# Ruyi-Zha/r2_gaussian

Hardware: NVIDIA H100
Metric: projections_per_sec (higher is better)
Workload: dtype f32

## Files before the change

### r2_gaussian_b200/csrc/r2x_api.cu

```cuda
#include <atomic>
#include <cstdio>
#include <cstring>
#include <string>
#include "../../include/r2x.h"
#include "r2x_binning.cuh"
#include "r2x_raster.cuh"
#include "r2x_voxel.cuh"

namespace r2x {
int launch_adam(cudaStream_t st, int ngroups, const r2x_adam_group* groups, double beta1, double beta2, double eps,
                long long step, const float* const* grads2, const uint32_t* guard0, const uint32_t* guard1);
int launch_densify_stats(cudaStream_t st, int P, const int* radii, const float* grad2d, float* max_radii, float* accum,
                         float* denom, const uint32_t* guard0, const uint32_t* guard1);

static thread_local std::string g_err;
static thread_local Activation g_act = {0, 0, 0.f, 0.f};
Activation current_activation() { return g_act; }
void set_activation(const Activation* a) { g_act = a ? *a : Activation{0, 0, 0.f, 0.f}; }

int fail(cudaError_t e, const char* what, const char* file, int line) {
    char buf[512];
    snprintf(buf, sizeof(buf), "CUDA error %d (%s) at %s:%d: %s", (int)e, cudaGetErrorString(e), file, line, what);
    g_err = buf;
    return R2X_ERR_CUDA;
// ... 227 lines not shown
    uint2* ranges = (uint2*)al((size_t)image_buf);
    if (P == 0) {
        R2X_CUDA_OK(cudaMemsetAsync(out_color, 0, sizeof(float) * (size_t)W * H, st));
        R2X_CUDA_OK(cudaMemsetAsync(ranges, 0, sizeof(uint2) * tiles, st));
        R2X_CUDA_OK(cudaMemsetAsync(s.status, 0, 16, st));
        if (status_dev) R2X_CUDA_OK(cudaMemsetAsync(status_dev, 0, 8, st));
        return 0;
    }
    if (!means3D || !opacities || !radii || !viewmatrix || !projmatrix)
        return fail_msg(R2X_ERR_INVALID, "r2x_raster_forward: null input");
    if (!cov3D_precomp && (!scales || !rotations))
        return fail_msg(R2X_ERR_INVALID, "r2x_raster_forward: need scales+rotations or cov3D_precomp");
    const bool direct = direct_ok(tiles);
    DirectBin db{};
    if (direct) {
        db = carve_directbin(image_buf, P, tiles);
    }
    R2X_TRY(launch_raster_preprocess(st, P, means3D, scales, scale_modifier, rotations, opacities, cov3D_precomp,
                                     viewmatrix, projmatrix, W, H, tan_fovx, tan_fovy, mode, prefiltered, radii,
                                     s.geom, direct ? &db : nullptr));
    R2X_TRY(debug_sync(st, debug, "raster preprocess"));
    if (direct) {
        const long long cap0 = binning_alloc ? (1ll << 62) : capacity;
        R2X_TRY(launch_direct_scan(st, db, s.status, cap0, binning_alloc ? nullptr : status_dev));
    } else {
        R2X_TRY(launch_scan(st, P, s.geom.tiles_touched, s.geom.offsets, s.scan_state, s.status));
    }
    R2X_TRY(debug_sync(st, debug, "raster scan"));
    long long R_launch;
    if (binning_alloc) {
        uint32_t R = 0;
        R2X_CUDA_OK(cudaMemcpyAsync(&R, s.status, sizeof(uint32_t), cudaMemcpyDeviceToHost, st));
        R2X_CUDA_OK(cudaStreamSynchronize(st));
        if (num_rendered) *num_rendered = (int)R;
        binning_buf = binning_alloc(binning_bytes((long long)R), alloc_user);
        if (!binning_buf) return fail_msg(R2X_ERR_INVALID, "r2x_raster_forward: binning allocator returned NULL");
        capacity = R;
        R_launch = R;
    } else {
        if (!binning_buf || capacity < 0) return fail_msg(R2X_ERR_INVALID, "r2x_raster_forward_async: no binning buffer");
        R_launch = capacity;
    }
    BinningView bv = binning_view(binning_buf, capacity);
    const TilePlan plan = carve_plan(image_buf, tiles, bv);
    if (direct) {
        R2X_TRY(launch_direct_fill(st, P, s.geom.cube, s.geom.tiles_touched, s.geom.offsets, db, ranges, plan, bv,
                                   s.geom.gx, s.geom.gy, s.status));
    } else {
        status_kernel<<<1, 1, 0, st>>>(s.status, capacity, status_dev);
        R2X_TRY(bin_instances(st, P, s.geom.cube, s.geom.tiles_touched, s.geom.offsets, s.geom.gx, s.geom.gy, tiles,
                              s.status, bv, R_launch, ranges));
        R2X_TRY(launch_plan(st, ranges, plan));
    }
    R2X_TRY(debug_sync(st, debug, "raster binning"));
    R2X_TRY(launch_raster_render(st, W, H, s.geom, ranges, bv.point_list, plan, R_launch, out_color));
    R2X_TRY(debug_sync(st, debug, "raster render"));
    return 0;
}

int voxel_forward_impl(cudaStream_t st, int P, int nx, int ny, int nz, float sx, float sy, float sz, float cx,
                       float cy, float cz, const float* means3D, const float* opacities, const float* scales,
                       float scale_modifier, const float* rotations, const float* cov3D_precomp, int prefiltered,
                       float* out_volume, int* radii_x, int* radii_y, int* radii_z, void* geom_buf, void* image_buf,
                       r2x_alloc_fn binning_alloc, void* alloc_user, void* binning_buf, long long capacity,
                       uint32_t* status_dev, int debug, int* num_rendered) {
    (void)prefiltered;
    if (nx <= 0 || ny <= 0 || nz <= 0 || P < 0) return fail_msg(R2X_ERR_INVALID, "r2x_voxel_forward: bad P/grid");
    if (!out_volume || !geom_buf || !image_buf) return fail_msg(R2X_ERR_INVALID, "r2x_voxel_forward: null output/state buffer");
    if (num_rendered) *num_rendered = 0;
    const VoxelGrid vg = make_voxel_grid(nx, ny, nz, sx, sy, sz, cx, cy, cz);
// ... 8 lines not shown
        R2X_CUDA_OK(cudaMemsetAsync(ranges, 0, sizeof(uint2) * (size_t)tiles, st));
        R2X_CUDA_OK(cudaMemsetAsync(s.status, 0, 16, st));
        if (status_dev) R2X_CUDA_OK(cudaMemsetAsync(status_dev, 0, 8, st));
        return 0;
    }
    if (!means3D || !opacities || !radii_x || !radii_y || !radii_z)
        return fail_msg(R2X_ERR_INVALID, "r2x_voxel_forward: null input");
    if (!scales)
        return fail_msg(R2X_ERR_INVALID,
                        "r2x_voxel_forward: scales are required (the bounding radius is 3*max(scale)/dVoxel even "
                        "with cov3D_precomp; the reference dereferences scales unconditionally, VOX/forward.cu:137)");
    if (!cov3D_precomp && !rotations) return fail_msg(R2X_ERR_INVALID, "r2x_voxel_forward: need rotations or cov3D_precomp");
    const bool direct = direct_ok(tiles);
    const bool two_level = two_level_ok(vg.gx, vg.gy, vg.gz);
    DirectBin db{};
    if (direct) {
        db = carve_directbin(image_buf, P, tiles);
    }
    R2X_TRY(launch_voxel_preprocess(st, P, means3D, scales, scale_modifier, rotations, opacities, cov3D_precomp, vg,
                                    radii_x, radii_y, radii_z, s.geom, direct ? &db : nullptr));
    R2X_TRY(debug_sync(st, debug, "voxel preprocess"));
    if (direct) {
        const long long cap0 = binning_alloc ? (1ll << 62) : capacity;
        R2X_TRY(launch_direct_scan(st, db, s.status, cap0, binning_alloc ? nullptr : status_dev));
    } else {
        R2X_TRY(launch_scan(st, P, s.geom.tiles_touched, s.geom.offsets, s.scan_state, s.status));
    }
    long long R_launch;
    if (binning_alloc) {
        uint32_t R = 0;
        R2X_CUDA_OK(cudaMemcpyAsync(&R, s.status, sizeof(uint32_t), cudaMemcpyDeviceToHost, st));
        R2X_CUDA_OK(cudaStreamSynchronize(st));
        if (num_rendered) *num_rendered = (int)R;
        binning_buf = binning_alloc(binning_bytes((long long)R), alloc_user);
        if (!binning_buf) return fail_msg(R2X_ERR_INVALID, "r2x_voxel_forward: binning allocator returned NULL");
        capacity = R;
        R_launch = R;
    } else {
        if (!binning_buf || capacity < 0) return fail_msg(R2X_ERR_INVALID, "r2x_voxel_forward_async: no binning buffer");
        R_launch = capacity;
    }
    BinningView bv = binning_view(binning_buf, capacity);
    const TilePlan plan = carve_voxel_plan(image_buf, tiles, bv);
    if (direct) {
        R2X_TRY(launch_direct_fill(st, P, s.geom.cube, s.geom.tiles_touched, s.geom.offsets, db, ranges, plan, bv, vg.gx,
                                   vg.gy, s.status));
    } else if (two_level) {
        status_kernel<<<1, 1, 0, st>>>(s.status, capacity, status_dev);
        const TwoLevel tl = carve_two_level(image_buf, P, vg.gx, vg.gy, vg.gz, bv);
        R2X_TRY(launch_two_level(st, P, s.geom.cube, s.geom.tiles_touched, vg.gx, vg.gy, vg.gz, s.status, tl, bv, ranges,
                                 plan));
    } else {
        status_kernel<<<1, 1, 0, st>>>(s.status, capacity, status_dev);
        R2X_TRY(bin_instances(st, P, s.geom.cube, s.geom.tiles_touched, s.geom.offsets, vg.gx, vg.gy, tiles, s.status,
                              bv, R_launch, ranges));
        R2X_TRY(launch_plan(st, ranges, plan));
    }
    R2X_TRY(debug_sync(st, debug, "voxel binning"));
    R2X_TRY(launch_voxel_render(st, vg, s.geom, ranges, bv.point_list, plan, R_launch, out_volume));
    R2X_TRY(debug_sync(st, debug, "voxel render"));
    return 0;
}

}
}

using namespace r2x;

extern "C" {
// ... 322 lines not shown
```

### r2_gaussian_b200/csrc/r2x_binning.cu

```cuda
#include <cstdlib>
#include "r2x_binning.cuh"

namespace r2x {

static inline size_t align_up(size_t v, size_t a) { return (v + a - 1) / a * a; }

static size_t plan_items(long long R) { return (size_t)(R > 0 ? R : 1) / PLAN_MIN_CHUNK + 1; }

int plan_chunk_override() {
    static int v = -1;
    if (v < 0) {
        const char* e = getenv("R2X_CHUNK");
        v = e ? atoi(e) : 0;
        if (v < 0) v = 0;
    }
    return v;
}

size_t binning_bytes(long long R) {
    size_t r = (size_t)(R > 0 ? R : 1);
    size_t per = align_up(r * sizeof(uint32_t), 256);
    return 7 * per + align_up(256 * SORT_MAX_BLOCKS * sizeof(uint32_t), 256) +
           align_up(plan_items(R) * sizeof(uint2), 256) + align_up(plan_items(R) * 512 * sizeof(float), 256) + 256;
}
// ... 416 lines not shown
    }
}

__global__ void __launch_bounds__(256) tile_ranges_kernel(const uint32_t* __restrict__ keys,
                                                          const uint32_t* __restrict__ d_total,
                                                          long long capacity, uint2* __restrict__ ranges) {
    long long R = *d_total;
    if (R > capacity) R = capacity;
    const long long stride = (long long)gridDim.x * blockDim.x;
    for (long long i = (long long)blockIdx.x * blockDim.x + threadIdx.x; i < R; i += stride) {
        const uint32_t cur = keys[i];
        if (i == 0) ranges[cur].x = 0;
        else {
            const uint32_t prev = keys[i - 1];
            if (cur != prev) { ranges[prev].y = (uint32_t)i; ranges[cur].x = (uint32_t)i; }
        }
        if (i == R - 1) ranges[cur].y = (uint32_t)R;
    }
}

size_t directbin_bytes(int P, int num_tiles) {
    const size_t nb = (size_t)((P > 0 ? P : 1) + DIRECT_BLOCK - 1) / DIRECT_BLOCK;
    const size_t t = (size_t)num_tiles;
    return align_up(t * nb * sizeof(uint32_t), 256) + align_up(t * sizeof(uint32_t), 256) +
           2 * align_up(nb * sizeof(uint32_t), 256) + 512;
}

DirectBin directbin_view(void* buf, int P, int num_tiles) {
    DirectBin db;
    const size_t nb = (size_t)((P > 0 ? P : 1) + DIRECT_BLOCK - 1) / DIRECT_BLOCK;
    const size_t t = (size_t)num_tiles;
    char* p = (char*)align_up((size_t)buf, 256);
    db.table = (uint32_t*)p; p += align_up(t * nb * sizeof(uint32_t), 256);
    db.tile_count = (uint32_t*)p; p += align_up(t * sizeof(uint32_t), 256);
    db.block_total = (uint32_t*)p; p += align_up(nb * sizeof(uint32_t), 256);
    db.block_base = (uint32_t*)p; p += align_up(nb * sizeof(uint32_t), 256);
    db.num_tiles = num_tiles;
    db.nb = (int)nb;
    return db;
}

template <typename Load, typename Store>
__device__ __forceinline__ uint32_t cta_exclusive_scan(int n, Load load, Store store, uint32_t* s_w, uint32_t* s_carry) {
    const int tid = threadIdx.x, lane = tid & 31, warp = tid >> 5;
    if (tid == 0) *s_carry = 0;
    __syncthreads();
    for (int base = 0; base < n; base += 256) {
        const int i = base + tid;
        const uint32_t a = i < n ? load(i) : 0u;
        uint32_t ia = a;
#pragma unroll
        for (int o = 1; o < 32; o <<= 1) {
            const uint32_t t = __shfl_up_sync(0xffffffffu, ia, o);
            if (lane >= o) ia += t;
        }
        if (lane == 31) s_w[warp] = ia;
        __syncthreads();
        uint32_t wpre = 0;
#pragma unroll
        for (int w = 0; w < 8; ++w)
            if (w < warp) wpre += s_w[w];
        const uint32_t ex = *s_carry + wpre + ia - a;
        if (i < n) store(i, ex, a);
        __syncthreads();
        if (tid == 255) *s_carry = ex + a;
        __syncthreads();
    }
    return *s_carry;
}

template <typename V, typename Load, typename Store>
__device__ __forceinline__ V cta_exclusive_scan_1pass(int n, Load load, Store store, V* s_w) {
    const int tid = threadIdx.x, lane = tid & 31, warp = tid >> 5;
    const int K = (n + 255) >> 8;
    V val[16], sum = 0;
#pragma unroll
    for (int k = 0; k < 16; ++k) {
        const int i = tid * K + k;
        val[k] = (k < K && i < n) ? load(i) : V(0);
        sum += val[k];
    }
    V ia = sum;
#pragma unroll
    for (int o = 1; o < 32; o <<= 1) {
        const V t = __shfl_up_sync(0xffffffffu, ia, o);
        if (lane >= o) ia += t;
    }
    __syncthreads();
    if (lane == 31) s_w[warp] = ia;
    __syncthreads();
    V wpre = 0, total = 0;
#pragma unroll
    for (int w = 0; w < 8; ++w) {
        const V x = s_w[w];
        if (w < warp) wpre += x;
        total += x;
    }
    V ex = wpre + ia - sum;
#pragma unroll
    for (int k = 0; k < 16; ++k) {
        const int i = tid * K + k;
        if (k < K && i < n) store(i, ex, val[k], total);
        ex += val[k];
    }
    return total;
}

constexpr int SCAN_SEGS = 32;
__global__ void __launch_bounds__(1024) direct_scan_kernel(DirectBin db, uint32_t* __restrict__ status,
                                                           long long capacity, uint32_t* __restrict__ status_out) {
    pdl_prologue();
    __shared__ uint32_t s_seg[SCAN_SEGS][33];
    __shared__ uint32_t s_red[32];
    const int lane = threadIdx.x & 31, seg = threadIdx.x >> 5;
    const int T = db.num_tiles, nb = db.nb;
    const int t = blockIdx.x * 32 + lane;
    const int rps = (nb + SCAN_SEGS - 1) / SCAN_SEGS;
    const int r0 = min(seg * rps, nb), r1 = min(r0 + rps, nb);
    uint32_t sum = 0;
    if (t < T) {
        const uint32_t* col = db.table + t;
        int r = r0;
        for (; r + 4 <= r1; r += 4) {
            const uint32_t a0 = col[(size_t)r * T], a1 = col[(size_t)(r + 1) * T], a2 = col[(size_t)(r + 2) * T],
                           a3 = col[(size_t)(r + 3) * T];
            sum += (a0 + a1) + (a2 + a3);
        }
        for (; r < r1; ++r) sum += col[(size_t)r * T];
    }
    s_seg[seg][lane] = sum;
    __syncthreads();
    uint32_t pre = 0;
    for (int k = 0; k < seg; ++k) pre += s_seg[k][lane];
    if (t < T) {
        if (seg == SCAN_SEGS - 1) db.tile_count[t] = pre + sum;
        uint32_t* col = db.table + t;
        int r = r0;
        for (; r + 4 <= r1; r += 4) {
            const uint32_t a0 = col[(size_t)r * T], a1 = col[(size_t)(r + 1) * T], a2 = col[(size_t)(r + 2) * T],
                           a3 = col[(size_t)(r + 3) * T];
            col[(size_t)r * T] = pre;
            col[(size_t)(r + 1) * T] = pre + a0;
            col[(size_t)(r + 2) * T] = pre + a0 + a1;
            col[(size_t)(r + 3) * T] = pre + a0 + a1 + a2;
            pre += (a0 + a1) + (a2 + a3);
        }
        for (; r < r1; ++r) {
            const uint32_t a = col[(size_t)r * T];
            col[(size_t)r * T] = pre;
            pre += a;
        }
    }
    if (blockIdx.x == 0) {
        __shared__ uint32_t s_carry;
        if (threadIdx.x == 0) s_carry = 0;
        __syncthreads();
        for (int base = 0; base < nb; base += 1024) {
            const int i = base + threadIdx.x;
            const uint32_t a = i < nb ? db.block_total[i] : 0u;
            uint32_t ia = a;
#pragma unroll
            for (int o = 1; o < 32; o <<= 1) {
                const uint32_t x = __shfl_up_sync(0xffffffffu, ia, o);
                if (lane >= o) ia += x;
            }
            if (lane == 31) s_red[seg] = ia;
            __syncthreads();
            uint32_t wpre = 0;
            for (int w = 0; w < seg; ++w) wpre += s_red[w];
            const uint32_t ex = s_carry + wpre + ia - a;
            if (i < nb) db.block_base[i] = ex;
            __syncthreads();
            if (threadIdx.x == 1023) s_carry = ex + a;
            __syncthreads();
        }
        if (threadIdx.x == 0) {
            const uint32_t R = s_carry;
            const uint32_t ov = ((long long)R > capacity) ? 1u : 0u;
            status[0] = R;
            status[1] = ov;
            if (status_out) { status_out[0] = R; status_out[1] = ov; }
        }
    }
}

int launch_direct_scan(cudaStream_t st, const DirectBin& db, uint32_t* status, long long capacity,
                       uint32_t* status_out) {
    R2X_CUDA_OK(pdl_launch(direct_scan_kernel, dim3((db.num_tiles + 31) / 32), dim3(1024), 0, st, db, status, capacity,
                           status_out));
    R2X_CUDA_OK(cudaGetLastError());
    return 0;
}

__global__ void __launch_bounds__(DIRECT_BLOCK) direct_fill_kernel(int P, const uint16_t* __restrict__ cube,
                                                                   const uint32_t* __restrict__ tiles_touched,
                                                                   uint32_t* __restrict__ offsets, DirectBin db,
                                                                   uint2* __restrict__ ranges, TilePlan pl,
                                                                   uint32_t* __restrict__ point_list,
                                                                   uint32_t* __restrict__ inst_pos, long long capacity,
                                                                   int gx, int gy, const uint32_t* __restrict__ status) {
    pdl_prologue();
    extern __shared__ __align__(16) unsigned char smem_raw[];
    __shared__ unsigned long long s_w[8];
    const int T = db.num_tiles;
    const int tid = threadIdx.x, lane = tid & 31, warp = tid >> 5;
    const uint32_t* tc = db.tile_count;
    uint32_t* s_mask = reinterpret_cast<uint32_t*>(smem_raw);
    uint32_t* s_base = s_mask + 8 * (size_t)T;
    unsigned char* s_wrank = reinterpret_cast<unsigned char*>(s_base + T);
    __shared__ uint32_t s_w8[8];

    const int b = blockIdx.x;
    const int g = b * DIRECT_BLOCK + tid;
    for (int i = tid; i < 2 * T; i += DIRECT_BLOCK) reinterpret_cast<uint4*>(s_mask)[i] = make_uint4(0u, 0u, 0u, 0u);
    uint32_t n = 0, c01 = 0, c23 = 0, c45 = 0;
    if (g < P) {
        n = tiles_touched[g];
        const uint32_t* c = reinterpret_cast<const uint32_t*>(cube + 6 * (size_t)g);
        c01 = c[0]; c23 = c[1]; c45 = c[2];
    }
    const uint32_t bbase = db.block_base[b];
    uint32_t ia = n;
#pragma unroll
    for (int o = 1; o < 32; o <<= 1) {
        const uint32_t x = __shfl_up_sync(0xffffffffu, ia, o);
        if (lane >= o) ia += x;
    }
    if (lane == 31) s_w8[warp] = ia;
    const uint32_t* row = db.table + (size_t)b * T;
    const uint32_t C = plan_chunk_for(status[0], pl.chunk_override, pl.chunk_cap);
    const int npub = db.nb < DIRECT_BLOCK ? db.nb : DIRECT_BLOCK;
    const bool pub = (b < npub) && (tid % npub == b);
    const unsigned long long tot = cta_exclusive_scan_1pass<unsigned long long>(
        T,
        [&](int i) {
            const uint32_t c = tc[i];
            return ((unsigned long long)(c ? (c - 1) / C : 0u) << 32) | c;
        },
        [&](int i, unsigned long long ex64, unsigned long long v64, unsigned long long total) {
            const uint32_t ex = (uint32_t)ex64, cnt = (uint32_t)v64;
            s_base[i] = ex + row[i];
            if (pub) {
                const bool ov = (long long)(uint32_t)total > capacity;
                const uint32_t eo = ov ? 0u : (uint32_t)(ex64 >> 32), ne = ov ? 0u : (uint32_t)(v64 >> 32);
                ranges[i] = ov ? make_uint2(0u, 0u) : make_uint2(ex, ex + cnt);
                pl.extra_off[i] = eo;
#pragma unroll
                for (int k = 0; k < PLAN_DONE_SLOTS; ++k) pl.tile_done[(size_t)i * PLAN_DONE_SLOTS + k] = 0;
                for (uint32_t c = 0; c < ne; ++c)
                    if ((long long)(eo + c) < pl.max_extra) pl.extra_item[eo + c] = make_uint2((uint32_t)i, c + 1);
            }
        },
        s_w);
    const uint32_t R = (uint32_t)tot;
    if (b == 0 && tid == 0) {
        pl.extra_off[T] = ((long long)R > capacity) ? 0u : (uint32_t)(tot >> 32);
        pl.counter[0] = pl.counter[1] = pl.counter[3] = 0;
        pl.counter[2] = C;
    }
    uint32_t wpre = 0;
#pragma unroll
    for (int w = 0; w < 8; ++w)
        if (w < warp) wpre += s_w8[w];
    const uint32_t lex = wpre + ia - n;
    if (g < P) offsets[g] = bbase + lex + n;
    if ((long long)R > capacity) return;
    const uint32_t x0 = c01 & 0xffff, y0 = c01 >> 16, z0 = c23 & 0xffff, x1 = c23 >> 16, y1 = c45 & 0xffff, z1 = c45 >> 16;
    {
        uint32_t* plane = s_mask + (size_t)warp * T;
        const uint32_t bit = 1u << lane;
        if (n)
            for (uint32_t z = z0; z < z1; ++z)
                for (uint32_t y = y0; y < y1; ++y) {
                    const uint32_t rowb = (z * (uint32_t)gy + y) * (uint32_t)gx;
                    for (uint32_t x = x0; x < x1; ++x) atomicOr(&plane[rowb + x], bit);
                }
    }
    __syncthreads();
    for (int t = tid; t < T; t += DIRECT_BLOCK) {
        uint32_t run = 0;
#pragma unroll
        for (int w = 0; w < 8; ++w) {
            s_wrank[(size_t)w * T + t] = (unsigned char)run;
            run += __popc(s_mask[(size_t)w * T + t]);
        }
    }
    __syncthreads();
    if (n) {
        const uint32_t* plane = s_mask + (size_t)warp * T;
        const unsigned char* wr = s_wrank + (size_t)warp * T;
        const uint32_t below = (1u << lane) - 1u;
        for (uint32_t z = z0; z < z1; ++z)
            for (uint32_t y = y0; y < y1; ++y) {
                const uint32_t rowb = (z * (uint32_t)gy + y) * (uint32_t)gx;
                for (uint32_t x = x0; x < x1; ++x) {
                    const uint32_t t = rowb + x;
                    const uint32_t pos = s_base[t] + wr[t] + __popc(plane[t] & below);
                    point_list[pos] = (uint32_t)g;
                }
            }
    }
}

int launch_direct_fill(cudaStream_t st, int P, const uint16_t* cube, const uint32_t* tiles_touched, uint32_t* offsets,
                       const DirectBin& db, uint2* ranges, const TilePlan& plan, const BinningView& bv, int gx,
                       int gy, const uint32_t* status) {
    const size_t smem = (size_t)db.num_tiles * 44;
    if (smem > 40 * 1024)
        R2X_CUDA_OK(cudaFuncSetAttribute(direct_fill_kernel, cudaFuncAttributeMaxDynamicSharedMemorySize,
                                         DIRECT_MAX_TILES * 44));
    R2X_CUDA_OK(pdl_launch(direct_fill_kernel, dim3(db.nb), dim3(DIRECT_BLOCK), smem, st, P, cube, tiles_touched, offsets,
                           db, ranges, plan, bv.point_list, bv.inst_pos, bv.capacity, gx, gy, status));
    R2X_CUDA_OK(cudaGetLastError());
    return 0;
}

int launch_sort_and_ranges(cudaStream_t st, long long R_launch, int num_tiles, const uint32_t* d_total,
                           const BinningView& bv, uint2* ranges, uint32_t** sorted_keys_out) {
    R2X_CUDA_OK(cudaMemsetAsync(ranges, 0, sizeof(uint2) * (size_t)num_tiles, st));
    if (sorted_keys_out) *sorted_keys_out = bv.keys[0];
    if (R_launch <= 0) return 0;
    int bits = 1;
    while ((1ll << bits) < (long long)num_tiles) ++bits;
    const int passes = (bits + 7) / 8;
    long long nbl = (R_launch + SORT_CHUNK - 1) / SORT_CHUNK;
    const int nb = (int)(nbl < SORT_MAX_BLOCKS ? nbl : SORT_MAX_BLOCKS);
    int cur = 0;
    for (int p = 0; p < passes; ++p) {
        const int shift = 8 * p;
        const bool first = (p == 0), last = (p == passes - 1);
        sort_hist_kernel<<<nb, SORT_THREADS, 0, st>>>(bv.keys[cur], d_total, bv.capacity, shift, nb, bv.hist);
        sort_scan_kernel<<<1, 1024, 0, st>>>(bv.hist, 256 * nb);
#define R2X_SCATTER(F, L)                                                                                          \
    sort_scatter_kernel<F, L><<<nb, SORT_THREADS, 0, st>>>(bv.keys[cur], bv.vals[cur], bv.keys[cur ^ 1],           \
                                                           bv.vals[cur ^ 1], bv.inst_g, bv.point_list, bv.inst_pos, \
// ... 21 lines not shown
```

### r2_gaussian_b200/csrc/r2x_binning.cuh

```cuda
#pragma once
#include "r2x_common.cuh"

namespace r2x {

struct BinningView {
    uint32_t* keys[2];
    uint32_t* vals[2];
    uint32_t* inst_g;
    uint32_t* point_list;
    uint32_t* inst_pos;
    uint32_t* hist;
    uint2* extra_item;
    float* partial;
    long long capacity;
};

constexpr int SORT_THREADS = 256;
constexpr int SORT_ITEMS = 16;
constexpr int SORT_CHUNK = SORT_THREADS * SORT_ITEMS;
constexpr int SORT_MAX_BLOCKS = 264;

constexpr int PLAN_CHUNK = 256;
constexpr int PLAN_MIN_CHUNK = 64;
constexpr int PLAN_DONE_SLOTS = 8;
// ... 35 lines not shown

__host__ __device__ __forceinline__ void plan_slice(const uint2 r, int chunk, int nch, uint32_t& begin, int& n) {
    const uint32_t len = r.y - r.x;
    const uint32_t q = len / (uint32_t)nch, rem = len - q * (uint32_t)nch;
    const uint32_t c = (uint32_t)chunk;
    begin = r.x + q * c + (c < rem ? c : rem);
    n = (int)(q + (c < rem ? 1u : 0u));
}

__device__ __forceinline__ void plan_decode(const TilePlan& pl, const uint2* __restrict__ ranges, uint32_t item,
                                            int& tile, int& chunk, int& nch, uint32_t& begin, int& n) {
    if ((int)item < pl.num_tiles) { tile = (int)item; chunk = 0; }
    else { const uint2 e = pl.extra_item[item - pl.num_tiles]; tile = (int)e.x; chunk = (int)e.y; }
    nch = (int)(pl.extra_off[tile + 1] - pl.extra_off[tile]) + 1;
    const uint2 r = ranges[tile];
    plan_slice(r, chunk, nch, begin, n);
}

size_t binning_bytes(long long R);
BinningView binning_view(void* buf, long long R);

constexpr int DIRECT_MAX_TILES = 4096;
constexpr int DIRECT_BLOCK = 256;
struct DirectBin {
    uint32_t* table;
    uint32_t* tile_count;
    uint32_t* block_total;
    uint32_t* block_base;
    int num_tiles, nb;
};
size_t directbin_bytes(int P, int num_tiles);
DirectBin directbin_view(void* buf, int P, int num_tiles);
inline bool direct_ok(int num_tiles) { return num_tiles <= DIRECT_MAX_TILES; }

__device__ __forceinline__ void block_tile_histogram(uint32_t* hist_s, const DirectBin& db, uint32_t c01, uint32_t c23,
                                                     uint32_t c45, uint32_t n, int gx, int gy) {
    const int tid = threadIdx.x;
    for (int t = tid; t < db.num_tiles; t += DIRECT_BLOCK) hist_s[t] = 0;
    __syncthreads();
    if (n) {
        const uint32_t x0 = c01 & 0xffff, y0 = c01 >> 16, z0 = c23 & 0xffff, x1 = c23 >> 16, y1 = c45 & 0xffff,
                       z1 = c45 >> 16;
        for (uint32_t z = z0; z < z1; ++z)
            for (uint32_t y = y0; y < y1; ++y) {
                const uint32_t rowb = (z * (uint32_t)gy + y) * (uint32_t)gx;
                for (uint32_t x = x0; x < x1; ++x) atomicAdd(&hist_s[rowb + x], 1u);
            }
    }
    __shared__ uint32_t s_wsum[DIRECT_BLOCK / 32];
    uint32_t v = n;
#pragma unroll
    for (int o = 16; o > 0; o >>= 1) v += __shfl_xor_sync(0xffffffffu, v, o);
    if ((tid & 31) == 0) s_wsum[tid >> 5] = v;
    __syncthreads();
    for (int t = tid; t < db.num_tiles; t += DIRECT_BLOCK) db.table[(size_t)blockIdx.x * db.num_tiles + t] = hist_s[t];
    if (tid == 0) {
        uint32_t tot = 0;
#pragma unroll
        for (int w = 0; w < DIRECT_BLOCK / 32; ++w) tot += s_wsum[w];
        db.block_total[blockIdx.x] = tot;
    }
// ... 2 lines not shown
struct TwoLevel {
    int gx1, gy1, gz1, T1;
    uint16_t* cube1;
    uint32_t* tiles1;
    uint32_t* offsets1;
    uint32_t* status1;
    uint2* ranges1;
    TilePlan plan1;
    DirectBin db1;
    uint32_t* list1;
    uint32_t* table2a;
    uint32_t* table2b;
    uint32_t* tile_count;
    uint32_t* tile_incl;
    void* scan_state;
};
bool two_level_ok(int gx, int gy, int gz);
size_t two_level_bytes(int P, int gx, int gy, int gz);
TwoLevel two_level_view(void* buf, int P, int gx, int gy, int gz, const BinningView& bv);
int launch_two_level(cudaStream_t st, int P, const uint16_t* cube, const uint32_t* tiles_touched, int gx, int gy, int gz,
                     const uint32_t* status, const TwoLevel& tl, const BinningView& bv, uint2* ranges,
                     const TilePlan& plan);

int launch_direct_scan(cudaStream_t st, const DirectBin& db, uint32_t* status, long long capacity,
                       uint32_t* status_out);
int launch_direct_fill(cudaStream_t st, int P, const uint16_t* cube, const uint32_t* tiles_touched, uint32_t* offsets,
                       const DirectBin& db, uint2* ranges, const TilePlan& plan, const BinningView& bv, int gx,
                       int gy, const uint32_t* status);

size_t scan_state_bytes(int P);
int launch_scan(cudaStream_t st, int P, const uint32_t* tiles_touched, uint32_t* offsets, void* scan_state,
                uint32_t* d_total);

int launch_emit(cudaStream_t st, int P, const uint16_t* cube, const uint32_t* tiles_touched,
                const uint32_t* offsets, int gx, int gy, const uint32_t* d_total, const BinningView& bv);

int launch_sort_and_ranges(cudaStream_t st, long long R_launch, int num_tiles, const uint32_t* d_total,
                           const BinningView& bv, uint2* ranges, uint32_t** sorted_keys_out);

size_t knn_scratch_bytes(int P);
int launch_knn3(cudaStream_t st, int P, const float* points, float* out, void* scratch, size_t scratch_bytes);

size_t image_loss_scratch_bytes(int H, int W);
int launch_image_loss(cudaStream_t st, int H, int W, const float* image, const float* target, float w_l1,
                      float w_dssim, float* loss_out, float* grad_out, void* scratch, size_t scratch_bytes);
size_t tv3d_scratch_bytes(int nx, int ny, int nz);
int launch_tv3d(cudaStream_t st, int nx, int ny, int nz, const float* vol, int reduction_mean, float* loss_out,
                float* grad_out, void* scratch, size_t scratch_bytes);

}
```

### r2_gaussian_b200/csrc/r2x_binning2.cu

```cuda
#include <cstdlib>
#include <cstring>

#include "r2x_binning.cuh"

#define R2X_PASS(expr)               \
    do {                             \
        const int rc_ = (expr);      \
        if (rc_) return rc_;         \
    } while (0)

namespace r2x {

namespace {

inline size_t align_up(size_t v, size_t a) { return (v + a - 1) / a * a; }

constexpr int SUP = 4;
constexpr int SUP_TILES = SUP * SUP * SUP;
constexpr int L2_CHUNK = PLAN_CHUNK;
static_assert(SUP_TILES == 64, "the membership of an entry is one 64-bit mask");
static_assert(L2_CHUNK == 256, "one thread per entry");

__device__ __forceinline__ void unpack_cube(const uint16_t* __restrict__ cube, uint32_t g, uint32_t& x0, uint32_t& y0,
                                            uint32_t& z0, uint32_t& x1, uint32_t& y1, uint32_t& z1) {
// ... 228 lines not shown
    b1.extra_item = reinterpret_cast<uint2*>(bv.vals[0]);
    b1.partial = nullptr;
    tl.plan1 = plan_view(q, tl.T1, b1); q += plan_bytes(tl.T1) + 256;
    tl.plan1.chunk_override = L2_CHUNK;
    tl.plan1.max_extra = bv.capacity / 2;
    tl.db1 = directbin_view(q, P, tl.T1); q += directbin_bytes(P, tl.T1) + 256;
    q = (char*)align_up((size_t)q, 256);
    tl.table2a = (uint32_t*)q; q += align_up((size_t)tl.T1 * SUP_TILES * sizeof(uint32_t), 256);
    tl.tile_count = (uint32_t*)q; q += align_up(T * sizeof(uint32_t), 256);
    tl.tile_incl = (uint32_t*)q; q += align_up(T * sizeof(uint32_t), 256);
    tl.scan_state = (void*)q;
    tl.list1 = bv.keys[0];
    tl.table2b = bv.keys[1];
    return tl;
}

int launch_two_level(cudaStream_t st, int P, const uint16_t* cube, const uint32_t* tiles_touched, int gx, int gy, int gz,
                     const uint32_t* status, const TwoLevel& tl, const BinningView& bv, uint2* ranges,
                     const TilePlan& plan) {
    const int T = gx * gy * gz;
    super_cube_kernel<<<tl.db1.nb, DIRECT_BLOCK, (size_t)tl.T1 * sizeof(uint32_t), st>>>(P, cube, tiles_touched, tl.cube1,
                                                                                          tl.tiles1, tl.db1, tl.gx1, tl.gy1);
    R2X_CUDA_OK(cudaGetLastError());
    R2X_PASS(launch_direct_scan(st, tl.db1, tl.status1, bv.capacity, nullptr));
    BinningView b1 = bv;
    b1.point_list = tl.list1;
    R2X_PASS(launch_direct_fill(st, P, tl.cube1, tl.tiles1, tl.offsets1, tl.db1, tl.ranges1, tl.plan1, b1, tl.gx1, tl.gy1,
                           tl.status1));
    int sms;
    R2X_CUDA_OK(sm_count(&sms));
    const int grid = sms * 4;
    fine_count_kernel<<<grid, L2_CHUNK, 0, st>>>(tl.plan1, tl.ranges1, tl.list1, cube, tl.gx1, tl.gy1, tl.table2a,
                                                 tl.table2b, status);
    fine_scan_kernel<<<tl.T1, SUP_TILES, 0, st>>>(tl.plan1, tl.table2a, tl.table2b, tl.gx1, tl.gy1, gx, gy, gz,
                                                  tl.tile_count, status);
    R2X_CUDA_OK(cudaGetLastError());
    R2X_PASS(launch_scan(st, T, tl.tile_count, tl.tile_incl, tl.scan_state, tl.status1 + 2));
    fine_ranges_kernel<<<(T + 255) / 256, 256, 0, st>>>(T, tl.tile_count, tl.tile_incl, status, ranges);
    R2X_CUDA_OK(cudaGetLastError());
    R2X_PASS(launch_plan(st, ranges, plan));
    fine_fill_kernel<<<grid, L2_CHUNK, 0, st>>>(tl.plan1, tl.ranges1, tl.list1, cube, tl.gx1, tl.gy1, gx, gy, gz,
                                                tl.table2a, tl.table2b, tl.tile_count, tl.tile_incl, status,
                                                bv.point_list);
    R2X_CUDA_OK(cudaGetLastError());
    return 0;
}

}
```

Baseline: 8005.

## Move tile ranges and plan into a decoupled-lookback direct scan; stage fill writes

The direct-binning scan kernel becomes a 256-thread, 8-column-per-CTA kernel that uses a decoupled lookback across CTAs. It computes per-tile ranges, plan extra offsets and tile_done resets itself, which removes that work from the fill kernel and drops the tile_count buffer. The fill kernel now stages point-list writes in shared memory when the per-block count fits, so the global scatter is done in a more ordered pass. The cost is more complex synchronisation (spin-wait lookback relying on dynamic block ids), more shared memory, and reordered setup that must stay consistent across the raster, voxel and two-level paths.

```diff
diff --git a/r2_gaussian_b200/csrc/r2x_api.cu b/r2_gaussian_b200/csrc/r2x_api.cu
--- a/r2_gaussian_b200/csrc/r2x_api.cu
+++ b/r2_gaussian_b200/csrc/r2x_api.cu
@@ -273,7 +273,8 @@
     R2X_TRY(debug_sync(st, debug, "raster preprocess"));
     if (direct) {
         const long long cap0 = binning_alloc ? (1ll << 62) : capacity;
-        R2X_TRY(launch_direct_scan(st, db, s.status, cap0, binning_alloc ? nullptr : status_dev));
+        R2X_TRY(launch_direct_scan(st, db, ranges, carve_plan(image_buf, tiles, BinningView{}), s.status, cap0,
+                                   binning_alloc ? nullptr : status_dev));
     } else {
         R2X_TRY(launch_scan(st, P, s.geom.tiles_touched, s.geom.offsets, s.scan_state, s.status));
     }
@@ -295,8 +296,8 @@
     BinningView bv = binning_view(binning_buf, capacity);
     const TilePlan plan = carve_plan(image_buf, tiles, bv);
     if (direct) {
-        R2X_TRY(launch_direct_fill(st, P, s.geom.cube, s.geom.tiles_touched, s.geom.offsets, db, ranges, plan, bv,
-                                   s.geom.gx, s.geom.gy, s.status));
+        R2X_TRY(launch_direct_fill(st, P, s.geom.cube, s.geom.tiles_touched, s.geom.offsets, db, plan, bv, s.geom.gx,
+                                   s.geom.gy, s.status));
     } else {
         status_kernel<<<1, 1, 0, st>>>(s.status, capacity, status_dev);
         R2X_TRY(bin_instances(st, P, s.geom.cube, s.geom.tiles_touched, s.geom.offsets, s.geom.gx, s.geom.gy, tiles,
@@ -351,7 +352,8 @@
     R2X_TRY(debug_sync(st, debug, "voxel preprocess"));
     if (direct) {
         const long long cap0 = binning_alloc ? (1ll << 62) : capacity;
-        R2X_TRY(launch_direct_scan(st, db, s.status, cap0, binning_alloc ? nullptr : status_dev));
+        R2X_TRY(launch_direct_scan(st, db, ranges, carve_voxel_plan(image_buf, tiles, BinningView{}), s.status,
+                                   cap0, binning_alloc ? nullptr : status_dev));
     } else {
         R2X_TRY(launch_scan(st, P, s.geom.tiles_touched, s.geom.offsets, s.scan_state, s.status));
     }
@@ -372,8 +374,8 @@
     BinningView bv = binning_view(binning_buf, capacity);
     const TilePlan plan = carve_voxel_plan(image_buf, tiles, bv);
     if (direct) {
-        R2X_TRY(launch_direct_fill(st, P, s.geom.cube, s.geom.tiles_touched, s.geom.offsets, db, ranges, plan, bv, vg.gx,
-                                   vg.gy, s.status));
+        R2X_TRY(launch_direct_fill(st, P, s.geom.cube, s.geom.tiles_touched, s.geom.offsets, db, plan, bv, vg.gx, vg.gy,
+                                   s.status));
     } else if (two_level) {
         status_kernel<<<1, 1, 0, st>>>(s.status, capacity, status_dev);
         const TwoLevel tl = carve_two_level(image_buf, P, vg.gx, vg.gy, vg.gz, bv);
diff --git a/r2_gaussian_b200/csrc/r2x_binning.cu b/r2_gaussian_b200/csrc/r2x_binning.cu
--- a/r2_gaussian_b200/csrc/r2x_binning.cu
+++ b/r2_gaussian_b200/csrc/r2x_binning.cu
@@ -462,7 +462,8 @@
 size_t directbin_bytes(int P, int num_tiles) {
     const size_t nb = (size_t)((P > 0 ? P : 1) + DIRECT_BLOCK - 1) / DIRECT_BLOCK;
     const size_t t = (size_t)num_tiles;
-    return align_up(t * nb * sizeof(uint32_t), 256) + align_up(t * sizeof(uint32_t), 256) +
+    return align_up(t * nb * sizeof(uint32_t), 256) +
+           align_up((size_t)(1 + direct_scan_ctas(num_tiles)) * sizeof(unsigned long long), 256) +
            2 * align_up(nb * sizeof(uint32_t), 256) + 512;
 }
 
@@ -472,7 +473,8 @@
     const size_t t = (size_t)num_tiles;
     char* p = (char*)align_up((size_t)buf, 256);
     db.table = (uint32_t*)p; p += align_up(t * nb * sizeof(uint32_t), 256);
-    db.tile_count = (uint32_t*)p; p += align_up(t * sizeof(uint32_t), 256);
+    db.lookback = (unsigned long long*)p;
+    p += align_up((size_t)(1 + direct_scan_ctas(num_tiles)) * sizeof(unsigned long long), 256);
     db.block_total = (uint32_t*)p; p += align_up(nb * sizeof(uint32_t), 256);
     db.block_base = (uint32_t*)p; p += align_up(nb * sizeof(uint32_t), 256);
     db.num_tiles = num_tiles;
@@ -480,179 +482,201 @@
     return db;
 }
 
-template <typename Load, typename Store>
-__device__ __forceinline__ uint32_t cta_exclusive_scan(int n, Load load, Store store, uint32_t* s_w, uint32_t* s_carry) {
+constexpr int DSCAN_THREADS = 256;
+constexpr int DSCAN_WARPS = DSCAN_THREADS / 32;
+constexpr int DSCAN_SEGS = DSCAN_THREADS / DSCAN_COLS;
+constexpr int DSCAN_KEEP = 16;
+static_assert(DSCAN_COLS == 8, "a warp is 4 row segments x 8 columns");
+constexpr unsigned long long LB_AGG = 1ull << 62, LB_INCL = 2ull << 62, LB_VALUE = (1ull << 62) - 1;
+
+__global__ void __launch_bounds__(DSCAN_THREADS) direct_scan_kernel(DirectBin db, uint2* __restrict__ ranges, TilePlan pl,
+                                                                    uint32_t* __restrict__ status, long long capacity,
+                                                                    uint32_t* __restrict__ status_out) {
+    pdl_prologue();
+    __shared__ uint32_t s_w[DSCAN_WARPS];
+    __shared__ uint32_t s_wcol[DSCAN_WARPS][DSCAN_COLS];
+    __shared__ uint32_t s_tot[DSCAN_COLS];
+    __shared__ uint32_t s_bid;
+    __shared__ unsigned long long s_excl;
     const int tid = threadIdx.x, lane = tid & 31, warp = tid >> 5;
-    if (tid == 0) *s_carry = 0;
-    __syncthreads();
-    for (int base = 0; base < n; base += 256) {
-        const int i = base + tid;
-        const uint32_t a = i < n ? load(i) : 0u;
-        uint32_t ia = a;
-#pragma unroll
-        for (int o = 1; o < 32; o <<= 1) {
-            const uint32_t t = __shfl_up_sync(0xffffffffu, ia, o);
-            if (lane >= o) ia += t;
-        }
-        if (lane == 31) s_w[warp] = ia;
-        __syncthreads();
-        uint32_t wpre = 0;
-#pragma unroll
-        for (int w = 0; w < 8; ++w)
-            if (w < warp) wpre += s_w[w];
-        const uint32_t ex = *s_carry + wpre + ia - a;
-        if (i < n) store(i, ex, a);
-        __syncthreads();
-        if (tid == 255) *s_carry = ex + a;
-        __syncthreads();
-    }
-    return *s_carry;
-}
-
-template <typename V, typename Load, typename Store>
-__device__ __forceinline__ V cta_exclusive_scan_1pass(int n, Load load, Store store, V* s_w) {
-    const int tid = threadIdx.x, lane = tid & 31, warp = tid >> 5;
-    const int K = (n + 255) >> 8;
-    V val[16], sum = 0;
-#pragma unroll
-    for (int k = 0; k < 16; ++k) {
+    const int T = db.num_tiles, nb = db.nb, nctas = gridDim.x;
+    if (tid == 0) s_bid = (uint32_t)atomicAdd(&db.lookback[0], 1ull);
+
+    const int K = (nb + DSCAN_THREADS - 1) / DSCAN_THREADS;
+    uint32_t mine = 0;
+    for (int k = 0; k < K; ++k) {
         const int i = tid * K + k;
-        val[k] = (k < K && i < n) ? load(i) : V(0);
-        sum += val[k];
-    }
-    V ia = sum;
+        if (i < nb) mine += db.block_total[i];
+    }
+    uint32_t incl = mine;
 #pragma unroll
     for (int o = 1; o < 32; o <<= 1) {
-        const V t = __shfl_up_sync(0xffffffffu, ia, o);
-        if (lane >= o) ia += t;
-    }
-    __syncthreads();
-    if (lane == 31) s_w[warp] = ia;
-    __syncthreads();
-    V wpre = 0, total = 0;
-#pragma unroll
-    for (int w = 0; w < 8; ++w) {
-        const V x = s_w[w];
-        if (w < warp) wpre += x;
-        total += x;
-    }
-    V ex = wpre + ia - sum;
-#pragma unroll
-    for (int k = 0; k < 16; ++k) {
-        const int i = tid * K + k;
-        if (k < K && i < n) store(i, ex, val[k], total);
-        ex += val[k];
-    }
-    return total;
-}
-
-constexpr int SCAN_SEGS = 32;
-__global__ void __launch_bounds__(1024) direct_scan_kernel(DirectBin db, uint32_t* __restrict__ status,
-                                                           long long capacity, uint32_t* __restrict__ status_out) {
-    pdl_prologue();
-    __shared__ uint32_t s_seg[SCAN_SEGS][33];
-    __shared__ uint32_t s_red[32];
-    const int lane = threadIdx.x & 31, seg = threadIdx.x >> 5;
-    const int T = db.num_tiles, nb = db.nb;
-    const int t = blockIdx.x * 32 + lane;
-    const int rps = (nb + SCAN_SEGS - 1) / SCAN_SEGS;
+        const uint32_t x = __shfl_up_sync(0xffffffffu, incl, o);
+        if (lane >= o) incl += x;
+    }
+    if (lane == 31) s_w[warp] = incl;
+    __syncthreads();
+    uint32_t R = 0, wpre = 0;
+#pragma unroll 8
+    for (int w = 0; w < DSCAN_WARPS; ++w) {
+        const uint32_t x = s_w[w];
+        wpre += (w < warp) ? x : 0u;
+        R += x;
+    }
+    const bool ov = (long long)R > capacity;
+    const uint32_t C = plan_chunk_for(R, pl.chunk_override, pl.chunk_cap);
+    if (blockIdx.x == 0) {
+        uint32_t run = wpre + incl - mine;
+        for (int k = 0; k < K; ++k) {
+            const int i = tid * K + k;
+            if (i < nb) {
+                const uint32_t v = db.block_total[i];
+                db.block_base[i] = run;
+                run += v;
+            }
+        }
+        if (tid == 0) {
+            status[0] = R;
+            status[1] = ov ? 1u : 0u;
+            if (status_out) { status_out[0] = R; status_out[1] = ov ? 1u : 0u; }
+            pl.counter[0] = pl.counter[1] = pl.counter[3] = 0;
+            pl.counter[2] = C;
+        }
+    }
+
+    const int bid = (int)s_bid;
+    const int col = tid & (DSCAN_COLS - 1), seg = tid / DSCAN_COLS;
+    const int t = bid * DSCAN_COLS + col;
+    const int rps = (nb + DSCAN_SEGS - 1) / DSCAN_SEGS;
     const int r0 = min(seg * rps, nb), r1 = min(r0 + rps, nb);
+    uint32_t* cp = db.table + t;
+    const bool live = t < T;
+    uint32_t keep[DSCAN_KEEP];
     uint32_t sum = 0;
-    if (t < T) {
-        const uint32_t* col = db.table + t;
-        int r = r0;
-        for (; r + 4 <= r1; r += 4) {
-            const uint32_t a0 = col[(size_t)r * T], a1 = col[(size_t)(r + 1) * T], a2 = col[(size_t)(r + 2) * T],
-                           a3 = col[(size_t)(r + 3) * T];
-            sum += (a0 + a1) + (a2 + a3);
-        }
-        for (; r < r1; ++r) sum += col[(size_t)r * T];
-    }
-    s_seg[seg][lane] = sum;
-    __syncthreads();
-    uint32_t pre = 0;
-    for (int k = 0; k < seg; ++k) pre += s_seg[k][lane];
-    if (t < T) {
-        if (seg == SCAN_SEGS - 1) db.tile_count[t] = pre + sum;
-        uint32_t* col = db.table + t;
-        int r = r0;
-        for (; r + 4 <= r1; r += 4) {
-            const uint32_t a0 = col[(size_t)r * T], a1 = col[(size_t)(r + 1) * T], a2 = col[(size_t)(r + 2) * T],
-                           a3 = col[(size_t)(r + 3) * T];
-            col[(size_t)r * T] = pre;
-            col[(size_t)(r + 1) * T] = pre + a0;
-            col[(size_t)(r + 2) * T] = pre + a0 + a1;
-            col[(size_t)(r + 3) * T] = pre + a0 + a1 + a2;
-            pre += (a0 + a1) + (a2 + a3);
-        }
-        for (; r < r1; ++r) {
-            const uint32_t a = col[(size_t)r * T];
-            col[(size_t)r * T] = pre;
-            pre += a;
-        }
-    }
-    if (blockIdx.x == 0) {
-        __shared__ uint32_t s_carry;
-        if (threadIdx.x == 0) s_carry = 0;
-        __syncthreads();
-        for (int base = 0; base < nb; base += 1024) {
-            const int i = base + threadIdx.x;
-            const uint32_t a = i < nb ? db.block_total[i] : 0u;
-            uint32_t ia = a;
-#pragma unroll
-            for (int o = 1; o < 32; o <<= 1) {
-                const uint32_t x = __shfl_up_sync(0xffffffffu, ia, o);
-                if (lane >= o) ia += x;
-            }
-            if (lane == 31) s_red[seg] = ia;
-            __syncthreads();
-            uint32_t wpre = 0;
-            for (int w = 0; w < seg; ++w) wpre += s_red[w];
-            const uint32_t ex = s_carry + wpre + ia - a;
-            if (i < nb) db.block_base[i] = ex;
-            __syncthreads();
-            if (threadIdx.x == 1023) s_carry = ex + a;
-            __syncthreads();
-        }
-        if (threadIdx.x == 0) {
-            const uint32_t R = s_carry;
-            const uint32_t ov = ((long long)R > capacity) ? 1u : 0u;
-            status[0] = R;
-            status[1] = ov;
-            if (status_out) { status_out[0] = R; status_out[1] = ov; }
-        }
-    }
-}
-
-int launch_direct_scan(cudaStream_t st, const DirectBin& db, uint32_t* status, long long capacity,
-                       uint32_t* status_out) {
-    R2X_CUDA_OK(pdl_launch(direct_scan_kernel, dim3((db.num_tiles + 31) / 32), dim3(1024), 0, st, db, status, capacity,
-                           status_out));
+#pragma unroll
+    for (int k = 0; k < DSCAN_KEEP; ++k) {
+        keep[k] = (live && r0 + k < r1) ? cp[(size_t)(r0 + k) * T] : 0u;
+        sum += keep[k];
+    }
+    if (live)
+        for (int r = r0 + DSCAN_KEEP; r < r1; ++r) sum += cp[(size_t)r * T];
+    uint32_t sincl = sum;
+#pragma unroll
+    for (int o = DSCAN_COLS; o < 32; o <<= 1) {
+        const uint32_t x = __shfl_up_sync(0xffffffffu, sincl, o);
+        if (lane >= o) sincl += x;
+    }
+    if (lane >= 32 - DSCAN_COLS) s_wcol[warp][col] = sincl;
+    __syncthreads();
+    uint32_t pre = sincl - sum, tot = 0;
+#pragma unroll 8
+    for (int w = 0; w < DSCAN_WARPS; ++w) {
+        const uint32_t x = s_wcol[w][col];
+        pre += (w < warp) ? x : 0u;
+        tot += x;
+    }
+    if (tid < DSCAN_COLS) s_tot[tid] = tot;
+    __syncthreads();
+    uint32_t cnt_before = 0, ext_before = 0, cnt_all = 0, ext_all = 0;
+#pragma unroll
+    for (int c = 0; c < DSCAN_COLS; ++c) {
+        const uint32_t n = s_tot[c];
+        const uint32_t e = n ? (n - 1) / C : 0u;
+        cnt_before += (c < col) ? n : 0u;
+        ext_before += (c < col) ? e : 0u;
+        cnt_all += n;
+        ext_all += e;
+    }
+
+    if (warp == 0) {
+        volatile unsigned long long* st = db.lookback + 1;
+        const unsigned long long agg = ((unsigned long long)ext_all << 32) | cnt_all;
+        unsigned long long excl = 0;
+        if (bid == 0) {
+            if (lane == 0) st[0] = LB_INCL | agg;
+        } else {
+            if (lane == 0) st[bid] = LB_AGG | agg;
+            int top = bid - 1;
+            while (true) {
+                const int q = top - lane;
+                const unsigned long long s = q >= 0 ? (unsigned long long)st[q] : LB_INCL;
+                const uint32_t incl_lanes = __ballot_sync(0xffffffffu, (s >> 62) == 2ull);
+                const uint32_t wait_lanes = __ballot_sync(0xffffffffu, (s >> 62) == 0ull);
+                const int stop = incl_lanes ? __ffs(incl_lanes) - 1 : 31;
+                const uint32_t upto = stop == 31 ? 0xffffffffu : ((2u << stop) - 1u);
+                if (wait_lanes & upto) continue;
+                unsigned long long v = (lane <= stop) ? (s & LB_VALUE) : 0ull;
+#pragma unroll
+                for (int o = 16; o > 0; o >>= 1) v += __shfl_xor_sync(0xffffffffu, v, o);
+                excl += v;
+                if (incl_lanes) break;
+                top -= 32;
+            }
+            if (lane == 0) st[bid] = LB_INCL | (excl + agg);
+        }
+        if (lane == 0) s_excl = excl;
+    }
+    __syncthreads();
+    const uint32_t start = (uint32_t)s_excl + cnt_before;
+    const uint32_t eoff = (uint32_t)(s_excl >> 32) + ext_before;
+    if (live) {
+        uint32_t pos = start + pre;
+#pragma unroll
+        for (int k = 0; k < DSCAN_KEEP; ++k)
+            if (r0 + k < r1) {
+                cp[(size_t)(r0 + k) * T] = pos;
+                pos += keep[k];
+            }
+        for (int r = r0 + DSCAN_KEEP; r < r1; ++r) {
+            const uint32_t a = cp[(size_t)r * T];
+            cp[(size_t)r * T] = pos;
+            pos += a;
+        }
+        if (seg == 0) {
+            ranges[t] = ov ? make_uint2(0u, 0u) : make_uint2(start, start + tot);
+            pl.extra_off[t] = ov ? 0u : eoff;
+        }
+    }
+    if (tid < DSCAN_COLS * PLAN_DONE_SLOTS) {
+        const size_t i = (size_t)bid * DSCAN_COLS * PLAN_DONE_SLOTS + tid;
+        if (i < (size_t)T * PLAN_DONE_SLOTS) pl.tile_done[i] = 0;
+    }
+    if (bid == nctas - 1 && tid == 0) pl.extra_off[T] = ov ? 0u : (uint32_t)(s_excl >> 32) + ext_all;
+}
+
+int launch_direct_scan(cudaStream_t st, const DirectBin& db, uint2* ranges, const TilePlan& plan, uint32_t* status,
+                       long long capacity, uint32_t* status_out) {
+    R2X_CUDA_OK(pdl_launch(direct_scan_kernel, dim3(direct_scan_ctas(db.num_tiles)), dim3(DSCAN_THREADS), 0, st, db,
+                           ranges, plan, status, capacity, status_out));
     R2X_CUDA_OK(cudaGetLastError());
     return 0;
 }
+
+constexpr int FILL_STAGE_TILES = 4 * DIRECT_BLOCK;
+constexpr int FILL_STAGE_CAP = 4608;
 
 __global__ void __launch_bounds__(DIRECT_BLOCK) direct_fill_kernel(int P, const uint16_t* __restrict__ cube,
                                                                    const uint32_t* __restrict__ tiles_touched,
                                                                    uint32_t* __restrict__ offsets, DirectBin db,
-                                                                   uint2* __restrict__ ranges, TilePlan pl,
-                                                                   uint32_t* __restrict__ point_list,
-                                                                   uint32_t* __restrict__ inst_pos, long long capacity,
-                                                                   int gx, int gy, const uint32_t* __restrict__ status) {
-    pdl_prologue();
+                                                                   TilePlan pl, uint32_t* __restrict__ point_list,
+                                                                   int gx, int gy, const uint32_t* __restrict__ status,
+                                                                   int stage_cap) {
     extern __shared__ __align__(16) unsigned char smem_raw[];
-    __shared__ unsigned long long s_w[8];
+    __shared__ uint32_t s_w8[8];
+    __shared__ uint32_t s_ct[4][8];
     const int T = db.num_tiles;
     const int tid = threadIdx.x, lane = tid & 31, warp = tid >> 5;
-    const uint32_t* tc = db.tile_count;
     uint32_t* s_mask = reinterpret_cast<uint32_t*>(smem_raw);
     uint32_t* s_base = s_mask + 8 * (size_t)T;
     unsigned char* s_wrank = reinterpret_cast<unsigned char*>(s_base + T);
-    __shared__ uint32_t s_w8[8];
+    uint32_t* s_loc = reinterpret_cast<uint32_t*>(s_wrank + 8 * (size_t)T);
+    uint32_t* s_pos = s_loc + T;
+    unsigned char* s_id = reinterpret_cast<unsigned char*>(s_pos + stage_cap);
+    for (int i = tid; i < 2 * T; i += DIRECT_BLOCK) reinterpret_cast<uint4*>(s_mask)[i] = make_uint4(0u, 0u, 0u, 0u);
+    pdl_prologue();
 
     const int b = blockIdx.x;
     const int g = b * DIRECT_BLOCK + tid;
-    for (int i = tid; i < 2 * T; i += DIRECT_BLOCK) reinterpret_cast<uint4*>(s_mask)[i] = make_uint4(0u, 0u, 0u, 0u);
     uint32_t n = 0, c01 = 0, c23 = 0, c45 = 0;
     if (g < P) {
         n = tiles_touched[g];
@@ -660,6 +684,9 @@
         c01 = c[0]; c23 = c[1]; c45 = c[2];
     }
     const uint32_t bbase = db.block_base[b];
+    const bool ov = status[1] != 0u;
+    const uint32_t* row = db.table + (size_t)b * T;
+    for (int t = tid; t < T; t += DIRECT_BLOCK) s_base[t] = row[t];
     uint32_t ia = n;
 #pragma unroll
     for (int o = 1; o < 32; o <<= 1) {
@@ -667,44 +694,25 @@
         if (lane >= o) ia += x;
     }
     if (lane == 31) s_w8[warp] = ia;
-    const uint32_t* row = db.table + (size_t)b * T;
-    const uint32_t C = plan_chunk_for(status[0], pl.chunk_override, pl.chunk_cap);
-    const int npub = db.nb < DIRECT_BLOCK ? db.nb : DIRECT_BLOCK;
-    const bool pub = (b < npub) && (tid % npub == b);
-    const unsigned long long tot = cta_exclusive_scan_1pass<unsigned long long>(
-        T,
-        [&](int i) {
-            const uint32_t c = tc[i];
-            return ((unsigned long long)(c ? (c - 1) / C : 0u) << 32) | c;
-        },
-        [&](int i, unsigned long long ex64, unsigned long long v64, unsigned long long total) {
-            const uint32_t ex = (uint32_t)ex64, cnt = (uint32_t)v64;
-            s_base[i] = ex + row[i];
-            if (pub) {
-                const bool ov = (long long)(uint32_t)total > capacity;
-                const uint32_t eo = ov ? 0u : (uint32_t)(ex64 >> 32), ne = ov ? 0u : (uint32_t)(v64 >> 32);
-                ranges[i] = ov ? make_uint2(0u, 0u) : make_uint2(ex, ex + cnt);
-                pl.extra_off[i] = eo;
-#pragma unroll
-                for (int k = 0; k < PLAN_DONE_SLOTS; ++k) pl.tile_done[(size_t)i * PLAN_DONE_SLOTS + k] = 0;
-                for (uint32_t c = 0; c < ne; ++c)
-                    if ((long long)(eo + c) < pl.max_extra) pl.extra_item[eo + c] = make_uint2((uint32_t)i, c + 1);
-            }
-        },
-        s_w);
-    const uint32_t R = (uint32_t)tot;
-    if (b == 0 && tid == 0) {
-        pl.extra_off[T] = ((long long)R > capacity) ? 0u : (uint32_t)(tot >> 32);
-        pl.counter[0] = pl.counter[1] = pl.counter[3] = 0;
-        pl.counter[2] = C;
-    }
-    uint32_t wpre = 0;
-#pragma unroll
-    for (int w = 0; w < 8; ++w)
-        if (w < warp) wpre += s_w8[w];
-    const uint32_t lex = wpre + ia - n;
-    if (g < P) offsets[g] = bbase + lex + n;
-    if ((long long)R > capacity) return;
+    __syncthreads();
+    uint32_t wpre = 0, total = 0;
+#pragma unroll
+    for (int w = 0; w < 8; ++w) {
+        const uint32_t x = s_w8[w];
+        wpre += (w < warp) ? x : 0u;
+        total += x;
+    }
+    if (g < P) offsets[g] = bbase + wpre + ia;
+    if (ov) return;
+    {
+        const int K = (T + (int)gridDim.x - 1) / (int)gridDim.x;
+        const int t1 = min(T, (b + 1) * K);
+        for (int t = b * K + tid; t < t1; t += DIRECT_BLOCK) {
+            const uint32_t eo = pl.extra_off[t], ne = pl.extra_off[t + 1] - eo;
+            for (uint32_t c = 0; c < ne; ++c)
+                if ((long long)(eo + c) < pl.max_extra) pl.extra_item[eo + c] = make_uint2((uint32_t)t, c + 1);
+        }
+    }
     const uint32_t x0 = c01 & 0xffff, y0 = c01 >> 16, z0 = c23 & 0xffff, x1 = c23 >> 16, y1 = c45 & 0xffff, z1 = c45 >> 16;
     {
         uint32_t* plane = s_mask + (size_t)warp * T;
@@ -717,13 +725,47 @@
                 }
     }
     __syncthreads();
-    for (int t = tid; t < T; t += DIRECT_BLOCK) {
+    auto word_ranks = [&](int t) -> uint32_t {
         uint32_t run = 0;
 #pragma unroll
         for (int w = 0; w < 8; ++w) {
             s_wrank[(size_t)w * T + t] = (unsigned char)run;
             run += __popc(s_mask[(size_t)w * T + t]);
         }
+        return run;
+    };
+    const bool staged = stage_cap > 0 && total <= (uint32_t)stage_cap;
+    if (staged) {
+        uint32_t cnt[4], inc[4];
+#pragma unroll
+        for (int k = 0; k < 4; ++k) {
+            const int t = k * DIRECT_BLOCK + tid;
+            cnt[k] = t < T ? word_ranks(t) : 0u;
+            inc[k] = cnt[k];
+#pragma unroll
+            for (int o = 1; o < 32; o <<= 1) {
+                const uint32_t x = __shfl_up_sync(0xffffffffu, inc[k], o);
+                if (lane >= o) inc[k] += x;
+            }
+            if (lane == 31) s_ct[k][warp] = inc[k];
+        }
+        __syncthreads();
+        uint32_t carry = 0;
+#pragma unroll
+        for (int k = 0; k < 4; ++k) {
+            uint32_t before = 0, all = 0;
+#pragma unroll
+            for (int w = 0; w < 8; ++w) {
+                const uint32_t x = s_ct[k][w];
+                before += (w < warp) ? x : 0u;
+                all += x;
+            }
+            const int t = k * DIRECT_BLOCK + tid;
+            if (t < T) s_loc[t] = carry + before + inc[k] - cnt[k];
+            carry += all;
+        }
+    } else {
+        for (int t = tid; t < T; t += DIRECT_BLOCK) word_ranks(t);
     }
     __syncthreads();
     if (n) {
@@ -735,22 +777,37 @@
                 const uint32_t rowb = (z * (uint32_t)gy + y) * (uint32_t)gx;
                 for (uint32_t x = x0; x < x1; ++x) {
                     const uint32_t t = rowb + x;
-                    const uint32_t pos = s_base[t] + wr[t] + __popc(plane[t] & below);
-                    point_list[pos] = (uint32_t)g;
+                    const uint32_t r = wr[t] + __popc(plane[t] & below);
+                    if (staged) {
+                        const uint32_t slot = s_loc[t] + r;
+                        s_pos[slot] = s_base[t] + r;
+                        s_id[slot] = (unsigned char)tid;
+                    } else {
+                        point_list[s_base[t] + r] = (uint32_t)g;
+                    }
                 }
             }
     }
+    if (staged) {
+        __syncthreads();
+        const uint32_t g0 = (uint32_t)b * DIRECT_BLOCK;
+        for (uint32_t i = tid; i < total; i += DIRECT_BLOCK) point_list[s_pos[i]] = g0 + s_id[i];
+    }
 }
 
 int launch_direct_fill(cudaStream_t st, int P, const uint16_t* cube, const uint32_t* tiles_touched, uint32_t* offsets,
-                       const DirectBin& db, uint2* ranges, const TilePlan& plan, const BinningView& bv, int gx,
-                       int gy, const uint32_t* status) {
-    const size_t smem = (size_t)db.num_tiles * 44;
-    if (smem > 40 * 1024)
+                       const DirectBin& db, const TilePlan& plan, const BinningView& bv, int gx, int gy,
+                       const uint32_t* status) {
+    static_assert(FILL_STAGE_TILES <= 4 * DIRECT_BLOCK, "the staging scan handles at most 4 tiles per thread");
+    static_assert(FILL_STAGE_TILES * 48 + FILL_STAGE_CAP * 5 <= DIRECT_MAX_TILES * 44, "one attribute covers both layouts");
+    const int T = db.num_tiles;
+    const int cap = T <= FILL_STAGE_TILES ? FILL_STAGE_CAP : 0;
+    const size_t smem = (size_t)T * (cap ? 48 : 44) + (size_t)cap * 5;
+    if (smem > 48 * 1024)
         R2X_CUDA_OK(cudaFuncSetAttribute(direct_fill_kernel, cudaFuncAttributeMaxDynamicSharedMemorySize,
                                          DIRECT_MAX_TILES * 44));
     R2X_CUDA_OK(pdl_launch(direct_fill_kernel, dim3(db.nb), dim3(DIRECT_BLOCK), smem, st, P, cube, tiles_touched, offsets,
-                           db, ranges, plan, bv.point_list, bv.inst_pos, bv.capacity, gx, gy, status));
+                           db, plan, bv.point_list, gx, gy, status, cap));
     R2X_CUDA_OK(cudaGetLastError());
     return 0;
 }
diff --git a/r2_gaussian_b200/csrc/r2x_binning.cuh b/r2_gaussian_b200/csrc/r2x_binning.cuh
--- a/r2_gaussian_b200/csrc/r2x_binning.cuh
+++ b/r2_gaussian_b200/csrc/r2x_binning.cuh
@@ -81,13 +81,15 @@
 
 constexpr int DIRECT_MAX_TILES = 4096;
 constexpr int DIRECT_BLOCK = 256;
+constexpr int DSCAN_COLS = 8;
 struct DirectBin {
     uint32_t* table;
-    uint32_t* tile_count;
+    unsigned long long* lookback;
     uint32_t* block_total;
     uint32_t* block_base;
     int num_tiles, nb;
 };
+__host__ __device__ __forceinline__ int direct_scan_ctas(int num_tiles) { return (num_tiles + DSCAN_COLS - 1) / DSCAN_COLS; }
 size_t directbin_bytes(int P, int num_tiles);
 DirectBin directbin_view(void* buf, int P, int num_tiles);
 inline bool direct_ok(int num_tiles) { return num_tiles <= DIRECT_MAX_TILES; }
@@ -96,6 +98,8 @@
                                                      uint32_t c45, uint32_t n, int gx, int gy) {
     const int tid = threadIdx.x;
     for (int t = tid; t < db.num_tiles; t += DIRECT_BLOCK) hist_s[t] = 0;
+    if (blockIdx.x == 0)
+        for (int i = tid; i <= direct_scan_ctas(db.num_tiles); i += DIRECT_BLOCK) db.lookback[i] = 0ull;
     __syncthreads();
     if (n) {
         const uint32_t x0 = c01 & 0xffff, y0 = c01 >> 16, z0 = c23 & 0xffff, x1 = c23 >> 16, y1 = c45 & 0xffff,
@@ -144,11 +148,11 @@
                      const uint32_t* status, const TwoLevel& tl, const BinningView& bv, uint2* ranges,
                      const TilePlan& plan);
 
-int launch_direct_scan(cudaStream_t st, const DirectBin& db, uint32_t* status, long long capacity,
-                       uint32_t* status_out);
+int launch_direct_scan(cudaStream_t st, const DirectBin& db, uint2* ranges, const TilePlan& plan, uint32_t* status,
+                       long long capacity, uint32_t* status_out);
 int launch_direct_fill(cudaStream_t st, int P, const uint16_t* cube, const uint32_t* tiles_touched, uint32_t* offsets,
-                       const DirectBin& db, uint2* ranges, const TilePlan& plan, const BinningView& bv, int gx,
-                       int gy, const uint32_t* status);
+                       const DirectBin& db, const TilePlan& plan, const BinningView& bv, int gx, int gy,
+                       const uint32_t* status);
 
 size_t scan_state_bytes(int P);
 int launch_scan(cudaStream_t st, int P, const uint32_t* tiles_touched, uint32_t* offsets, void* scan_state,
diff --git a/r2_gaussian_b200/csrc/r2x_binning2.cu b/r2_gaussian_b200/csrc/r2x_binning2.cu
--- a/r2_gaussian_b200/csrc/r2x_binning2.cu
+++ b/r2_gaussian_b200/csrc/r2x_binning2.cu
@@ -274,11 +274,11 @@
     super_cube_kernel<<<tl.db1.nb, DIRECT_BLOCK, (size_t)tl.T1 * sizeof(uint32_t), st>>>(P, cube, tiles_touched, tl.cube1,
                                                                                           tl.tiles1, tl.db1, tl.gx1, tl.gy1);
     R2X_CUDA_OK(cudaGetLastError());
-    R2X_PASS(launch_direct_scan(st, tl.db1, tl.status1, bv.capacity, nullptr));
+    R2X_PASS(launch_direct_scan(st, tl.db1, tl.ranges1, tl.plan1, tl.status1, bv.capacity, nullptr));
     BinningView b1 = bv;
     b1.point_list = tl.list1;
-    R2X_PASS(launch_direct_fill(st, P, tl.cube1, tl.tiles1, tl.offsets1, tl.db1, tl.ranges1, tl.plan1, b1, tl.gx1, tl.gy1,
-                           tl.status1));
+    R2X_PASS(launch_direct_fill(st, P, tl.cube1, tl.tiles1, tl.offsets1, tl.db1, tl.plan1, b1, tl.gx1, tl.gy1,
+                                tl.status1));
     int sms;
     R2X_CUDA_OK(sm_count(&sms));
     const int grid = sms * 4;
```

Measured after the change: 8745 (median of 6 runs). 9.2% higher.
